# bytedance/ps-lite

Measured on AMD Instinct MI355X. Metric: push+pull GB/s per worker + p50 round-trip µs, 1 MB & 64 MB, at 1/2/4/8 GPUs, higher is better.
Workload: dtype fp32; 1 GPU; model=dense push+pull (ps-lite test_benchmark PUSH_PULL), global_batch=128, seq_len=67108864, parallelism=byteps-joint x1 (worker+server per GPU), mode=dense, msg_bytes=67108864, batch_keys=False, overlap=True, op=assign

## Files before the change

### csrc/kernels.h

```cpp
#pragma once

#include <cstddef>
#include <cstdint>

#include <hip/hip_runtime.h>

#include "coalesce_admit.h"

namespace xps {
namespace kern {

void DenseAssign(void* dst, const void* src, size_t nbytes, hipStream_t s, int grid_cap = 0);
void DenseAssign2(void* dst0, void* dst1, const void* src, size_t nbytes, hipStream_t s,
                  int grid_cap = 0);
inline bool Disjoint3(const void* a, const void* b, const void* c, size_t len) {
  auto apart = [len](const void* x, const void* y) {
    uintptr_t p = reinterpret_cast<uintptr_t>(x), q = reinterpret_cast<uintptr_t>(y);
    return p + len <= q || q + len <= p;
  };
  return apart(a, b) && apart(a, c) && apart(b, c);
}
void DenseSumF32(float* dst, const float* src, size_t n, hipStream_t s, int grid_cap = 0);
void DenseSumBf16(uint16_t* dst, const uint16_t* src, size_t n, hipStream_t s, int grid_cap = 0);
void BatchedSumBf16(const struct CopyDesc* descs_host, int n, hipStream_t s, int tile_cap = 0);
void SparseGatherF32(const float* table, const uint64_t* rows_dev, size_t nrows, size_t row_len,
                     float* out, hipStream_t s, int key_shift = 0, uint64_t row_base = 0,
                     uint64_t table_rows = ~0ull, int grid_cap = 0);
void SparseScatterAddF32(float* table, const uint64_t* rows_dev, size_t nrows, size_t row_len,
                         const float* src, bool atomic, hipStream_t s, int key_shift = 0,
                         uint64_t row_base = 0, uint64_t table_rows = ~0ull, int grid_cap = 0);
void SparseScatterAssignF32(float* table, const uint64_t* rows_dev, size_t nrows, size_t row_len,
                            const float* src, hipStream_t s, int key_shift = 0,
                            uint64_t row_base = 0, uint64_t table_rows = ~0ull,
                            int grid_cap = 0);

static const int kMaxBatch = 64;
struct CopyDesc {
  void* dst;
  const void* src;
  size_t nbytes;
};
void BatchedAssign(const CopyDesc* descs_host, int n, hipStream_t s, int tile_cap = 0);
void BatchedSumF32(const CopyDesc* descs_host, int n, hipStream_t s, int tile_cap = 0);

static_assert(kMaxBatch2 == kMaxBatch, "Seg2 batches use the batched kernels' segment limit");
void BatchedAssign2(const Seg2* segs_host, int n, hipStream_t s, int tile_cap = 0);

}
}
```

### csrc/kernels.hip

```cpp
#include <hip/hip_runtime.h>

#include <algorithm>
#include <cstdlib>

#include "kernels.h"
#include "tile_runs.h"

namespace xps {
namespace kern {

namespace {

constexpr int kBlock = 256;

inline int GridFor(size_t work_items, int cap = 8192) {
  size_t g = (work_items + kBlock - 1) / kBlock;
  if (g > static_cast<size_t>(cap)) g = cap;
  if (g == 0) g = 1;
  return static_cast<int>(g);
}

inline int CapGrid(int grid, int cap) { return cap > 0 && grid > cap ? cap : grid; }

__global__ void assign_kernel(uint4* __restrict__ dst, const uint4* __restrict__ src, size_t n4) {
  size_t i = blockIdx.x * static_cast<size_t>(blockDim.x) + threadIdx.x;
  size_t stride = static_cast<size_t>(gridDim.x) * blockDim.x;
  for (; i < n4; i += stride) dst[i] = src[i];
}

__global__ void assign_tail_kernel(char* __restrict__ dst, const char* __restrict__ src,
                                   size_t begin, size_t end) {
  size_t i = begin + blockIdx.x * static_cast<size_t>(blockDim.x) + threadIdx.x;
  size_t stride = static_cast<size_t>(gridDim.x) * blockDim.x;
  for (; i < end; i += stride) dst[i] = src[i];
}

__global__ void assign2_kernel(uint4* __restrict__ dst0, uint4* __restrict__ dst1,
                               const uint4* __restrict__ src, size_t n4, size_t tail_begin,
                               size_t nbytes) {
  size_t tid = blockIdx.x * static_cast<size_t>(blockDim.x) + threadIdx.x;
  size_t stride = static_cast<size_t>(gridDim.x) * blockDim.x;
  for (size_t i = tid; i < n4; i += stride) {
    uint4 v = src[i];
    dst0[i] = v;
    dst1[i] = v;
  }
  char* b0 = reinterpret_cast<char*>(dst0);
  char* b1 = reinterpret_cast<char*>(dst1);
  const char* bs = reinterpret_cast<const char*>(src);
  for (size_t i = tail_begin + tid; i < nbytes; i += stride) {
    char c = bs[i];
    b0[i] = c;
    b1[i] = c;
  }
}

__global__ void sum_kernel_f32(float4* __restrict__ dst, const float4* __restrict__ src,
                               size_t n4) {
  size_t i = blockIdx.x * static_cast<size_t>(blockDim.x) + threadIdx.x;
  size_t stride = static_cast<size_t>(gridDim.x) * blockDim.x;
  for (; i < n4; i += stride) {
    float4 d = dst[i];
    float4 s = src[i];
    d.x += s.x;
    d.y += s.y;
    d.z += s.z;
    d.w += s.w;
    dst[i] = d;
  }
}

__global__ void sum_tail_f32(float* __restrict__ dst, const float* __restrict__ src, size_t begin,
                             size_t end) {
  size_t i = begin + blockIdx.x * static_cast<size_t>(blockDim.x) + threadIdx.x;
  size_t stride = static_cast<size_t>(gridDim.x) * blockDim.x;
  for (; i < end; i += stride) dst[i] += src[i];
}

__device__ inline float bf16_to_f32(uint16_t h) {
  union {
    uint32_t u;
    float f;
  } c;
  c.u = static_cast<uint32_t>(h) << 16;
  return c.f;
}

// ... 58 lines not shown
                                     const float4* __restrict__ src, int shift, uint64_t base,
                                     uint64_t tab_rows) {
  size_t total = nrows * row_len4;
  size_t i = blockIdx.x * static_cast<size_t>(blockDim.x) + threadIdx.x;
  size_t stride = static_cast<size_t>(gridDim.x) * blockDim.x;
  for (; i < total; i += stride) {
    size_t r = i / row_len4;
    size_t c = i - r * row_len4;
    uint64_t row = (rows[r] >> shift) - base;
    if (row >= tab_rows) continue;
    float4* dst = table + row * row_len4 + c;
    float4 d = *dst;
    float4 v = src[i];
    d.x += v.x;
    d.y += v.y;
    d.z += v.z;
    d.w += v.w;
    *dst = d;
  }
}

__global__ void gather_rows_scalar_f32(const float* __restrict__ table,
                                       const uint64_t* __restrict__ rows, size_t nrows,
                                       size_t row_len, float* __restrict__ out, int shift,
                                       uint64_t base, uint64_t tab_rows) {
  for (size_t r = blockIdx.x; r < nrows; r += gridDim.x) {
    uint64_t row = (rows[r] >> shift) - base;
    const float* src = table + row * row_len;
    float* dst = out + r * row_len;
    for (size_t c = threadIdx.x; c < row_len; c += blockDim.x) {
      dst[c] = row < tab_rows ? src[c] : 0.f;
    }
  }
}

__global__ void scatter_assign_rows_f32(float4* __restrict__ table,
                                        const uint64_t* __restrict__ rows, size_t nrows,
                                        size_t row_len4, const float4* __restrict__ src,
                                        int shift, uint64_t base, uint64_t tab_rows) {
  size_t total = nrows * row_len4;
  size_t i = blockIdx.x * static_cast<size_t>(blockDim.x) + threadIdx.x;
  size_t stride = static_cast<size_t>(gridDim.x) * blockDim.x;
  for (; i < total; i += stride) {
    size_t r = i / row_len4;
    size_t c = i - r * row_len4;
    uint64_t row = (rows[r] >> shift) - base;
    if (row < tab_rows) table[row * row_len4 + c] = src[i];
  }
}

__global__ void scatter_assign_rows_scalar_f32(float* __restrict__ table,
                                               const uint64_t* __restrict__ rows, size_t nrows,
                                               size_t row_len, const float* __restrict__ src,
                                               int shift, uint64_t base, uint64_t tab_rows) {
  for (size_t r = blockIdx.x; r < nrows; r += gridDim.x) {
    uint64_t row = (rows[r] >> shift) - base;
    if (row >= tab_rows) continue;
    float* dst = table + row * row_len;
    const float* s = src + r * row_len;
    for (size_t c = threadIdx.x; c < row_len; c += blockDim.x) dst[c] = s[c];
  }
}

__global__ void scatter_add_rows_atomic_f32(float* __restrict__ table,
                                            const uint64_t* __restrict__ rows, size_t nrows,
                                            size_t row_len, const float* __restrict__ src,
                                            int shift, uint64_t base, uint64_t tab_rows) {
  for (size_t r = blockIdx.x; r < nrows; r += gridDim.x) {
    uint64_t row = (rows[r] >> shift) - base;
    if (row >= tab_rows) continue;
    float* dst = table + row * row_len;
    const float* s = src + r * row_len;
    for (size_t c = threadIdx.x; c < row_len; c += blockDim.x) {
      atomicAdd(&dst[c], s[c]);
    }
  }
}

struct DescArray {
  CopyDesc d[kMaxBatch];
  int n;
};

struct BalancedDescArray {
  CopyDesc d[kMaxBatch];
  unsigned long long prefix[kMaxBatch + 1];
  int n;
};

template <int kOp>
__global__ void batched_balanced_kernel(BalancedDescArray da, size_t chunks_per_block) {
  size_t total = da.prefix[da.n];
  size_t tile_begin = blockIdx.x * chunks_per_block;
  size_t tile_end = tile_begin + chunks_per_block;
  if (tile_end > total) tile_end = total;
  if (tile_begin >= total) return;
  int seg = 0;
  {
    int lo = 0, hi = da.n - 1;
    while (lo < hi) {
      int mid = (lo + hi + 1) >> 1;
      if (da.prefix[mid] <= tile_begin) {
        lo = mid;
      } else {
        hi = mid - 1;
      }
    }
    seg = lo;
  }
  for (size_t g = tile_begin + threadIdx.x; g < tile_end; g += blockDim.x) {
    while (g >= da.prefix[seg + 1]) ++seg;
    size_t local = g - da.prefix[seg];
    if (kOp == 1) {
      float4* dst = reinterpret_cast<float4*>(da.d[seg].dst) + local;
      const float4* src = reinterpret_cast<const float4*>(da.d[seg].src) + local;
      float4 a = *dst;
      float4 b = *src;
      a.x += b.x;
      a.y += b.y;
      a.z += b.z;
      a.w += b.w;
      *dst = a;
    } else if (kOp == 2) {
      uint4* dst = reinterpret_cast<uint4*>(da.d[seg].dst) + local;
      const uint4* src = reinterpret_cast<const uint4*>(da.d[seg].src) + local;
      uint4 a = *dst;
      uint4 b = *src;
      a.x = bf16x2_sum(a.x, b.x);
      a.y = bf16x2_sum(a.y, b.y);
      a.z = bf16x2_sum(a.z, b.z);
      a.w = bf16x2_sum(a.w, b.w);
      *dst = a;
    } else {
      reinterpret_cast<uint4*>(da.d[seg].dst)[local] =
          reinterpret_cast<const uint4*>(da.d[seg].src)[local];
    }
  }
}

struct Seg2Array {
  Seg2 d[kMaxBatch];
  unsigned long long prefix[kMaxBatch + 1];
  int n;
};

constexpr size_t kTileChunks2 = 512;

__global__ void __launch_bounds__(kBlock)
    batched_assign2_kernel(Seg2Array da, size_t chunks_per_block) {
  TileRunIter it = TileRunsBegin(da.prefix, da.n, chunks_per_block, blockIdx.x);
  TileRun run;
  while (TileRunsNext(da.prefix, &it, &run)) {
    uint4* __restrict__ d0 = static_cast<uint4*>(da.d[run.seg].dst0);
    uint4* __restrict__ d1 = static_cast<uint4*>(da.d[run.seg].dst1);
    const uint4* __restrict__ sp = static_cast<const uint4*>(da.d[run.seg].src);
    for (size_t i = run.lo + threadIdx.x; i < run.hi; i += kBlock) {
      uint4 v = sp[i];
      d0[i] = v;
      d1[i] = v;
    }
  }
}

__global__ void batched_assign_kernel(DescArray da) {
  for (int seg = 0; seg < da.n; ++seg) {
    uint4* dst = reinterpret_cast<uint4*>(da.d[seg].dst);
    const uint4* src = reinterpret_cast<const uint4*>(da.d[seg].src);
    size_t n4 = da.d[seg].nbytes / 16;
    size_t i = blockIdx.x * static_cast<size_t>(blockDim.x) + threadIdx.x;
    size_t stride = static_cast<size_t>(gridDim.x) * blockDim.x;
    for (; i < n4; i += stride) dst[i] = src[i];
  }
}

__global__ void batched_sum_kernel_bf16(DescArray da) {
  for (int seg = 0; seg < da.n; ++seg) {
    uint4* dst = reinterpret_cast<uint4*>(da.d[seg].dst);
    const uint4* src = reinterpret_cast<const uint4*>(da.d[seg].src);
    size_t n8 = da.d[seg].nbytes / 16;
    size_t i = blockIdx.x * static_cast<size_t>(blockDim.x) + threadIdx.x;
    size_t stride = static_cast<size_t>(gridDim.x) * blockDim.x;
    for (; i < n8; i += stride) {
      uint4 d = dst[i];
      uint4 s = src[i];
      d.x = bf16x2_sum(d.x, s.x);
      d.y = bf16x2_sum(d.y, s.y);
      d.z = bf16x2_sum(d.z, s.z);
      d.w = bf16x2_sum(d.w, s.w);
      dst[i] = d;
    }
  }
}

__global__ void batched_sum_kernel_f32(DescArray da) {
  for (int seg = 0; seg < da.n; ++seg) {
    float4* dst = reinterpret_cast<float4*>(da.d[seg].dst);
    const float4* src = reinterpret_cast<const float4*>(da.d[seg].src);
    size_t n4 = da.d[seg].nbytes / 16;
    size_t i = blockIdx.x * static_cast<size_t>(blockDim.x) + threadIdx.x;
    size_t stride = static_cast<size_t>(gridDim.x) * blockDim.x;
    for (; i < n4; i += stride) {
      float4 d = dst[i];
      float4 v = src[i];
      d.x += v.x;
      d.y += v.y;
      d.z += v.z;
      d.w += v.w;
      dst[i] = d;
    }
  }
}

}

namespace {

bool BalancedBatchEnabled() {
  static const bool on = [] {
    const char* v = getenv("XPS_BALANCED_BATCH");
    return !v || atoi(v) != 0;
  }();
  return on;
}

template <int kOp>
void LaunchBalanced(const CopyDesc* descs_host, int n, hipStream_t s, int tile_cap) {
  size_t max_blocks = tile_cap > 0 ? std::min(tile_cap, 8192) : 8192;
  for (int off = 0; off < n; off += kMaxBatch) {
    BalancedDescArray da{};
    da.n = std::min(n - off, kMaxBatch);
    unsigned long long acc = 0;
    for (int i = 0; i < da.n; ++i) {
      da.d[i] = descs_host[off + i];
      da.prefix[i] = acc;
      acc += da.d[i].nbytes / 16;
    }
    da.prefix[da.n] = acc;
    if (acc == 0) continue;
    size_t cpb = (acc + max_blocks - 1) / max_blocks;
    cpb = ((cpb + kBlock - 1) / kBlock) * kBlock;
    int grid = static_cast<int>((acc + cpb - 1) / cpb);
    hipLaunchKernelGGL((batched_balanced_kernel<kOp>), dim3(grid), dim3(kBlock), 0, s, da,
                       cpb);
  }
}

template <typename Kernel>
void LaunchLegacy(Kernel kernel, const CopyDesc* descs_host, int n, hipStream_t s,
                  int tile_cap) {
  size_t total = 0;
  for (int i = 0; i < n; ++i) total += descs_host[i].nbytes;
  if (total < 16) return;
  int grid = CapGrid(GridFor(total / 16), tile_cap);
  DescArray da{};
  for (int off = 0; off < n; off += kMaxBatch) {
    da.n = std::min(n - off, kMaxBatch);
    for (int i = 0; i < da.n; ++i) da.d[i] = descs_host[off + i];
    hipLaunchKernelGGL(kernel, dim3(grid), dim3(kBlock), 0, s, da);
  }
}

inline bool Aligned16(const void* a, const void* b) {
  return ((reinterpret_cast<uintptr_t>(a) | reinterpret_cast<uintptr_t>(b)) & 15u) == 0;
}

}

void BatchedAssign(const CopyDesc* descs_host, int n, hipStream_t s, int tile_cap) {
  if (BalancedBatchEnabled()) {
    LaunchBalanced<0>(descs_host, n, s, tile_cap);
    return;
  }
  LaunchLegacy(batched_assign_kernel, descs_host, n, s, tile_cap);
}

void BatchedAssign2(const Seg2* segs_host, int n, hipStream_t s, int tile_cap) {
  int max_blocks = tile_cap > 0 ? std::min(tile_cap, 8192) : 8192;
  int off = 0;
  while (off < n) {
    Seg2Array da{};
    unsigned long long acc = 0;
    while (off < n && da.n < kMaxBatch) {
      const Seg2& sg = segs_host[off++];
      if (sg.nbytes < 16) continue;
      da.d[da.n] = sg;
      da.prefix[da.n] = acc;
      acc += sg.nbytes / 16;
      ++da.n;
    }
    da.prefix[da.n] = acc;
    if (acc == 0) continue;
    size_t cpb = (acc + max_blocks - 1) / max_blocks;
    cpb = ((cpb + kBlock - 1) / kBlock) * kBlock;
    if (tile_cap <= 0 && cpb > kTileChunks2) cpb = kTileChunks2;
    int grid = static_cast<int>((acc + cpb - 1) / cpb);
    hipLaunchKernelGGL(batched_assign2_kernel, dim3(grid), dim3(kBlock), 0, s, da, cpb);
  }
}

void BatchedSumF32(const CopyDesc* descs_host, int n, hipStream_t s, int tile_cap) {
  if (BalancedBatchEnabled()) {
    LaunchBalanced<1>(descs_host, n, s, tile_cap);
    return;
  }
  LaunchLegacy(batched_sum_kernel_f32, descs_host, n, s, tile_cap);
}

void DenseAssign(void* dst, const void* src, size_t nbytes, hipStream_t s, int grid_cap) {
  if (!Aligned16(dst, src)) {
    if (nbytes == 0) return;
    hipLaunchKernelGGL(assign_tail_kernel, dim3(CapGrid(GridFor(nbytes), grid_cap)),
                       dim3(kBlock), 0, s, static_cast<char*>(dst),
                       static_cast<const char*>(src), size_t{0}, nbytes);
    return;
  }
  size_t n4 = nbytes / 16;
  if (n4) {
    hipLaunchKernelGGL(assign_kernel, dim3(CapGrid(GridFor(n4), grid_cap)), dim3(kBlock), 0, s,
                       static_cast<uint4*>(dst), static_cast<const uint4*>(src), n4);
  }
  if (nbytes % 16) {
    hipLaunchKernelGGL(assign_tail_kernel, dim3(1), dim3(kBlock), 0, s, static_cast<char*>(dst),
                       static_cast<const char*>(src), n4 * 16, nbytes);
  }
}

void DenseAssign2(void* dst0, void* dst1, const void* src, size_t nbytes, hipStream_t s,
                  int grid_cap) {
  if (nbytes == 0) return;
  bool aligned = ((reinterpret_cast<uintptr_t>(dst0) | reinterpret_cast<uintptr_t>(dst1) |
                   reinterpret_cast<uintptr_t>(src)) & 15u) == 0;
  size_t n4 = aligned ? nbytes / 16 : 0;
  int grid = GridFor(n4 ? n4 : nbytes);
  if (grid_cap > 0 && grid > grid_cap) grid = grid_cap;
  hipLaunchKernelGGL(assign2_kernel, dim3(grid), dim3(kBlock), 0, s, static_cast<uint4*>(dst0),
                     static_cast<uint4*>(dst1), static_cast<const uint4*>(src), n4, n4 * 16,
                     nbytes);
}

void DenseSumF32(float* dst, const float* src, size_t n, hipStream_t s, int grid_cap) {
  if (!Aligned16(dst, src)) {
    if (n == 0) return;
    hipLaunchKernelGGL(sum_tail_f32, dim3(CapGrid(GridFor(n), grid_cap)), dim3(kBlock), 0, s, dst,
                       src, size_t{0}, n);
    return;
  }
  size_t n4 = n / 4;
  if (n4) {
    hipLaunchKernelGGL(sum_kernel_f32, dim3(CapGrid(GridFor(n4), grid_cap)), dim3(kBlock), 0, s,
// ... 84 lines not shown
```

### csrc/pybind.cc

```cpp
#include <pybind11/functional.h>
#include <pybind11/numpy.h>
#include <pybind11/pybind11.h>
#include <pybind11/stl.h>

#include <atomic>
#include <thread>

#include "gpu_plane.h"
#include "hip_pool.h"
#include "hip_util.h"
#include "host_pool.h"
#include "kernels.h"
#include "kv_app.h"
#include "kv_utils.h"
#include "ps.h"
#include "server_handlers.h"
#include "shm_ring.h"
#include "simple_app.h"
#include "tile_runs.h"
#include "van.h"
#include "wire.h"

namespace py = pybind11;
using namespace xps;

namespace {

struct PoolBuffer {
  SArray<char> arr;
  uintptr_t ptr() const { return reinterpret_cast<uintptr_t>(arr.data()); }
  size_t nbytes() const { return arr.size(); }
  int device() const { return arr.device(); }
  void copy_from(py::array src) {
    py::buffer_info info = src.request();
    size_t n = static_cast<size_t>(info.size) * info.itemsize;
    XPS_CHECK_LE(n, arr.size());
    if (arr.on_device()) {
      gpu::CopyHostToDevice(arr.data(), info.ptr, n, arr.device());
    } else {
      memcpy(arr.data(), info.ptr, n);
    }
  }
  py::array_t<float> to_numpy_f32() const {
    size_t n = arr.size() / sizeof(float);
    py::array_t<float> out(n);
    if (arr.on_device()) {
      gpu::CopyDeviceToHost(out.mutable_data(), arr.data(), n * sizeof(float));
    } else {
      memcpy(out.mutable_data(), arr.data(), n * sizeof(float));
    }
    return out;
  }
};

class PyKVWorker {
 public:
  PyKVWorker(int app_id, int customer_id, int instance_idx)
      : w_(app_id, customer_id, instance_idx) {}

  int Push(py::array_t<uint64_t> keys, py::array_t<float> vals, py::array_t<int> lens) {
    SArray<Key> k;
    k.CopyFrom(keys.data(), keys.size());
    SArray<float> v;
    v.CopyFrom(vals.data(), vals.size());
    SArray<int> l;
    if (lens.size()) l.CopyFrom(lens.data(), lens.size());
    py::gil_scoped_release rel;
    return w_.ZPush(k, v, l);
  }

  py::array_t<float> PullBlocking(py::array_t<uint64_t> keys) {
    std::vector<Key> k(keys.data(), keys.data() + keys.size());
    std::vector<float> vals;
    std::vector<int> lens;
    {
      py::gil_scoped_release rel;
      int ts = w_.Pull(k, &vals, &lens);
      w_.Wait(ts);
    }
    py::array_t<float> out(vals.size());
    std::copy(vals.begin(), vals.end(), out.mutable_data());
    return out;
  }

  int ZPushPtr(py::array_t<uint64_t> keys, uintptr_t vals_ptr, size_t vals_bytes, int device,
               py::array_t<int> lens, int cmd, uintptr_t keys_dev_ptr) {
    SArray<Key> k;
    k.CopyFrom(keys.data(), keys.size());
    SArray<float> v(reinterpret_cast<float*>(vals_ptr), vals_bytes / sizeof(float), device);
    SArray<int> l;
    if (lens.size()) l.CopyFrom(lens.data(), lens.size());
    SArray<Key> kd;
    if (keys_dev_ptr) {
      kd = SArray<Key>(reinterpret_cast<Key*>(keys_dev_ptr), keys.size(), device);
    }
    py::gil_scoped_release rel;
    return w_.ZPush(k, v, l, cmd, nullptr, kd);
  }

  int ZPushPullPtr(py::array_t<uint64_t> keys, uintptr_t vals_ptr, uintptr_t out_ptr,
                   size_t vals_bytes, int device, py::array_t<int> lens, int cmd,
// ... 364 lines not shown
  m.def("kernel_on_stream", [](uintptr_t stream, uintptr_t dst, uintptr_t src, size_t n) {
    py::gil_scoped_release rel;
    kern::DenseSumF32(reinterpret_cast<float*>(dst), reinterpret_cast<float*>(src), n,
                      reinterpret_cast<hipStream_t>(stream));
    hipEvent_t ev;
    XPS_CHECK(hipEventCreateWithFlags(&ev, hipEventDisableTiming) == hipSuccess);
    XPS_CHECK(hipEventRecord(ev, reinterpret_cast<hipStream_t>(stream)) == hipSuccess);
    while (hipEventQuery(ev) != hipSuccess) {}
    (void)hipEventDestroy(ev);
  });
  m.def("ipc_open", [](py::bytes handle) {
    std::string h = handle;
    py::gil_scoped_release rel;
    hipIpcMemHandle_t hh;
    memcpy(&hh, h.data(), sizeof(hh));
    void* ptr = nullptr;
    hipError_t e = hipIpcOpenMemHandle(&ptr, hh, hipIpcMemLazyEnablePeerAccess);
    XPS_CHECK(e == hipSuccess) << "hipIpcOpenMemHandle: " << hipGetErrorString(e);
    return reinterpret_cast<uintptr_t>(ptr);
  });
  m.def("pool_in_use", []() { return HbmPool::Get()->bytes_in_use(); });
  m.def("pool_contains", [](uintptr_t p) {
    uint64_t off = 0;
    return HbmPool::Get()->OffsetOf(reinterpret_cast<const void*>(p), &off);
  });
  py::class_<PoolBuffer>(m, "PoolBuffer")
      .def_property_readonly("ptr", &PoolBuffer::ptr)
      .def_property_readonly("nbytes", &PoolBuffer::nbytes)
      .def_property_readonly("device", &PoolBuffer::device)
      .def("copy_from", &PoolBuffer::copy_from)
      .def("to_numpy_f32", &PoolBuffer::to_numpy_f32);
  m.def("pool_alloc", [](size_t nbytes) {
    PoolBuffer b;
    b.arr = HbmPool::Get()->AllocArray(nbytes);
    return b;
  });
  m.def("host_alloc", [](size_t nbytes) {
    PoolBuffer b;
    b.arr = HostShmPool::Get()->AllocArray(nbytes);
    return b;
  });

  py::class_<PyKVWorker>(m, "KVWorker")
      .def(py::init<int, int, int>(), py::arg("app_id") = 0, py::arg("customer_id") = 0,
           py::arg("instance_idx") = 0)
      .def("push", &PyKVWorker::Push, py::arg("keys"), py::arg("vals"),
           py::arg("lens") = py::array_t<int>())
      .def("pull", &PyKVWorker::PullBlocking, py::arg("keys"))
      .def("zpush_ptr", &PyKVWorker::ZPushPtr, py::arg("keys"), py::arg("vals_ptr"),
           py::arg("vals_bytes"), py::arg("device"), py::arg("lens") = py::array_t<int>(),
           py::arg("cmd") = 0, py::arg("keys_dev_ptr") = 0)
      .def("zpushpull_ptr", &PyKVWorker::ZPushPullPtr, py::arg("keys"), py::arg("vals_ptr"),
           py::arg("out_ptr"), py::arg("nbytes"), py::arg("device") = -1,
           py::arg("lens") = py::array_t<int>(), py::arg("cmd") = 0,
           py::arg("keys_dev_ptr") = 0)
      .def("zpull_ptr", &PyKVWorker::ZPullPtr, py::arg("keys"), py::arg("vals_ptr"),
           py::arg("vals_bytes"), py::arg("device"), py::arg("lens") = py::array_t<int>(),
           py::arg("cmd") = 0, py::arg("keys_dev_ptr") = 0)
      .def("wait", &PyKVWorker::Wait)
      .def("round", &PyKVWorker::Round, py::arg("keys"), py::arg("ptrs"), py::arg("nbytes"),
           py::arg("device"), py::arg("cmd") = 0, py::arg("pull") = false)
      .def("round_mixed", &PyKVWorker::RoundMixed, py::arg("keys"), py::arg("push_ptrs"),
           py::arg("pull_ptrs"), py::arg("sizes"), py::arg("device"), py::arg("cmd") = 0,
           py::arg("overlap") = true);

  py::class_<PyKVServer>(m, "KVServer")
      .def(py::init<int, int>(), py::arg("app_id") = 0, py::arg("instance_idx") = 0)
      .def("set_default_handle", &PyKVServer::SetDefaultHandle)
      .def("set_reduce_handle", &PyKVServer::SetReduceHandle, py::arg("num_workers"))
      .def("set_gpu_dense_handle", &PyKVServer::SetGpuDenseHandle, py::arg("mode") = "assign",
           py::arg("dtype") = "f32")
      .def("set_gpu_sparse_handle", &PyKVServer::SetGpuSparseHandle, py::arg("rows"),
           py::arg("row_len"), py::arg("accumulate") = true, py::arg("key_shift") = 0)
      .def("register_entry", &PyKVServer::RegisterEntry, py::arg("key"), py::arg("ptr"),
           py::arg("nbytes"), py::arg("device") = 0)
      .def("sparse_table_ptr", &PyKVServer::SparseTablePtr)
      .def("save_checkpoint", &PyKVServer::SaveCheckpoint)
      .def("load_checkpoint", &PyKVServer::LoadCheckpoint)
      .def("set_python_handle", &PyKVServer::SetPythonHandle);

  m.def("zero_copy_recv_count", []() { return g_zero_copy_recv.load(); });
  m.def("fused_assign_count", []() { return g_fused_assign.load(); });
  m.def("fused_assign_launches", []() { return g_fused_launches.load(); });
  m.def("coalesce_admit",
        [](const std::vector<std::tuple<uintptr_t, uintptr_t, uintptr_t, size_t>>& open,
           const std::tuple<uintptr_t, uintptr_t, uintptr_t, size_t>& seg) {
          auto conv = [](const std::tuple<uintptr_t, uintptr_t, uintptr_t, size_t>& t) {
            return kern::Seg2{reinterpret_cast<void*>(std::get<0>(t)),
                              reinterpret_cast<void*>(std::get<1>(t)),
                              reinterpret_cast<const void*>(std::get<2>(t)), std::get<3>(t)};
          };
          std::vector<kern::Seg2> segs;
          for (auto& t : open) segs.push_back(conv(t));
          switch (kern::CoalesceAdmit(segs.data(), static_cast<int>(segs.size()), conv(seg))) {
            case kern::Admit::kAdmit: return "admit";
            case kern::Admit::kFlushFirst: return "flush";
            default: return "reject";
          }
        },
        py::arg("open"), py::arg("seg"));
  m.def("tile_runs",
        [](const std::vector<unsigned long long>& chunk_counts,
           unsigned long long chunks_per_block, unsigned long long block_index) {
          if (chunks_per_block == 0) throw std::invalid_argument("tile_runs: empty tile");
          std::vector<unsigned long long> prefix(chunk_counts.size() + 1, 0);
          for (size_t i = 0; i < chunk_counts.size(); ++i) {
            if (chunk_counts[i] == 0) throw std::invalid_argument("tile_runs: empty segment");
            prefix[i + 1] = prefix[i] + chunk_counts[i];
          }
          int n = static_cast<int>(chunk_counts.size());
          std::vector<std::tuple<int, unsigned long long, unsigned long long>> out;
          kern::TileRunIter it = kern::TileRunsBegin(prefix.data(), n, chunks_per_block,
                                                     block_index);
          kern::TileRun run;
          while (kern::TileRunsNext(prefix.data(), &it, &run)) {
            out.emplace_back(run.seg, run.lo, run.hi);
          }
          return out;
        },
        py::arg("chunk_counts"), py::arg("chunks_per_block"), py::arg("block_index"));

  m.def("plane_peer_bytes", [](const std::string& role, int idx) {
    py::dict out;
    auto* po = GetPO(role, idx);
    auto* plane = po->van() ? dynamic_cast<GpuPlane*>(po->van()->plane()) : nullptr;
    if (plane) {
      for (auto& t : plane->PeerBytes()) {
        out[py::int_(std::get<0>(t))] = py::make_tuple(std::get<1>(t), std::get<2>(t));
      }
    }
    return out;
  }, py::arg("role") = "worker", py::arg("idx") = 0);

  m.def("_order_nodes", [](std::vector<std::tuple<std::string, std::string, int>> in) {
    std::vector<Node> nodes;
    for (auto& t : in) {
      Node n;
      n.role = std::get<0>(t) == "worker" ? Node::WORKER : Node::SERVER;
      n.hostname = std::get<1>(t);
      n.port = std::get<2>(t);
      nodes.push_back(n);
    }
    auto less = NodeRankOrder(nodes);
    std::sort(nodes.begin(), nodes.end(), less);
    std::vector<std::tuple<std::string, std::string, int>> out;
    for (auto& n : nodes) {
      out.emplace_back(n.role == Node::WORKER ? "worker" : "server", n.hostname, n.port);
    }
    return out;
  });

  m.def("_host_pool_init_for_test", [](uint64_t uid, size_t bytes) {
    HostShmPool::Get()->Init(uid, bytes);
  });
  m.def("_gc_stale_shm", []() { HostShmPool::GcStaleSegments(); });

  m.def("_ring_stress", [](int producers, int per, int payload) {
    ShmRing ring;
    XPS_CHECK(ring.Create(0xabcdef12345ull + getpid()));
    std::atomic<long> received{0}, sum{0}, pushed{0};
    std::atomic<bool> done{false};
    std::thread consumer([&]() {
      std::vector<char> buf(ShmRing::MaxPayload());
      while (true) {
        uint32_t n = ring.Pop(buf.data());
        if (n == 0) {
// ... 301 lines not shown
```

### csrc/server_handlers.cc

```cpp
#include "server_handlers.h"

#include "gpu_plane.h"
#include "hip_pool.h"
#include "kernels.h"

namespace xps {

#define XPS_HIP_CHECK(cmd)                                                            \
  do {                                                                                \
    hipError_t e_ = (cmd);                                                            \
    XPS_CHECK(e_ == hipSuccess) << "HIP error: " << hipGetErrorString(e_) << " in " #cmd; \
  } while (0)

static GpuPlane* ThePlane(Postoffice* po) {
  return dynamic_cast<GpuPlane*>(po->van() ? po->van()->plane() : nullptr);
}

static hipStream_t PeerStream(Postoffice* po, int sender, hipStream_t* fallback) {
  auto* plane = ThePlane(po);
  if (plane) return plane->StreamForPeer(sender);
  if (!*fallback) {
    XPS_HIP_CHECK(hipStreamCreateWithFlags(fallback, hipStreamNonBlocking));
  }
  return *fallback;
// ... 126 lines not shown
  }
  if (e->buf.size() != len) return false;
  const char* src = reinterpret_cast<const char*>(kvs.vals.data());
  if (!kern::Disjoint3(e->buf.data(), dst, src, len)) return false;
  bool chain = NeedChain(req.sender);
  bool coalesced = !chain && !e->last_ev &&
                   plane->CoalesceAppend(req.sender, kern::Seg2{e->buf.data(), dst, src, len});
  if (!coalesced) {
    hipStream_t stream = Stream(req.sender);
    OrderAfter(e, stream);
    kern::DenseAssign2(e->buf.data(), dst, src, len, stream);
    g_fused_launches.fetch_add(1, std::memory_order_relaxed);
    if (chain) e->last_ev = MakeEventRef(po_, stream);
  }
  g_fused_assign.fetch_add(1, std::memory_order_relaxed);
  g_zero_copy_recv.fetch_add(1, std::memory_order_relaxed);
  KVMeta r = req;
  r.option |= kOptInPlace;
  r.option &= ~(kOptPullLane | kOptEntryPush);
  r.val_len = static_cast<int64_t>(len);
  uint64_t eoff = 0;
  if (HbmPool::Get()->OffsetOf(e->buf.data(), &eoff)) {
    r.entry_addr = eoff;
    r.option |= kOptEntryAddr;
  }
  server->Response(r);
  if (coalesced) plane->CoalesceEnd(req.sender);
  return true;
}

GpuDenseHandler::Group* GpuDenseHandler::GroupFor(const SArray<Key>& keys) {
  uint64_t h = 1469598103934665603ull;
  const unsigned char* p = reinterpret_cast<const unsigned char*>(keys.data());
  for (size_t i = 0; i < keys.nbytes(); ++i) {
    h ^= p[i];
    h *= 1099511628211ull;
  }
  Group* g;
  {
    std::lock_guard<std::mutex> lk(mu_);
    g = &groups_[h];
  }
  if (g->keys.empty()) {
    g->keys.assign(keys.begin(), keys.end());
    g->ents.reserve(keys.size());
    std::lock_guard<std::mutex> lk(mu_);
    for (Key k : g->keys) g->ents.push_back(&store_[k]);
  } else {
    XPS_CHECK(g->keys.size() == keys.size() &&
              std::equal(g->keys.begin(), g->keys.end(), keys.begin()))
        << "reduce mode needs a consistent key->message grouping across workers "
           "(key-set hash collision or inconsistent bucketing)";
  }
  return g;
}

void GpuDenseHandler::HandleReducePush(const KVMeta& req, const KVPairs<float>& kvs,
                                       KVServer<float>* server) {
  XPS_STAGE(reduce_push);
  size_t n = kvs.keys.size();
  Group* g = GroupFor(kvs.keys);
  if (g->pushes >= num_workers_) {
    g->waiting_pushes.emplace_back(req, kvs);
    return;
  }
  XPS_CHECK(kvs.vals.on_device()) << "reduce mode needs device vals (pool buffers)";
  if (g->lens.size() != n) {
    g->lens.resize(n);
    for (size_t i = 0; i < n; ++i) {
      g->lens[i] = kvs.lens.empty() ? kvs.vals.nbytes() / n
                                    : static_cast<size_t>(kvs.lens[i]) * sizeof(float);
    }
  }
  hipStream_t stream = Stream(req.sender);
  XPS_HIP_CHECK(hipSetDevice(HbmPool::Get()->device()));
  if (g->last_ev) XPS_HIP_CHECK(hipStreamWaitEvent(stream, g->last_ev.get(), 0));
  bool first = g->pushes == 0;
  if (first) {
    for (auto& ev : g->pull_guard) {
      XPS_HIP_CHECK(hipStreamWaitEvent(stream, ev.get(), 0));
    }
    g->pull_guard.clear();
  }
  std::vector<kern::CopyDesc> descs;
  descs.reserve(n);
  size_t off = 0;
  bool aligned = true;
  for (size_t i = 0; i < n; ++i) {
    size_t len = g->lens[i];
    Entry* e = g->ents[i];
    if (e->buf.size() < len) e->buf = HbmPool::Get()->AllocArray(len);
    descs.push_back({e->buf.data(), reinterpret_cast<const char*>(kvs.vals.data()) + off, len});
    aligned = aligned && (len % 16 == 0);
    off += len;
  }
  if (aligned) {
    if (first) {
      kern::BatchedAssign(descs.data(), static_cast<int>(n), stream);
    } else {
      BatchedSum(descs.data(), static_cast<int>(n), stream);
    }
  } else {
    for (auto& d : descs) {
      if (first) {
        kern::DenseAssign(d.dst, d.src, d.nbytes, stream);
      } else {
        SumKernel(d.dst, d.src, d.nbytes, stream);
      }
    }
  }
  g->pushes++;
  EventRef ev = MakeEventRef(po_, stream);
  g->round_events.push_back(ev);
  g->last_ev = ev;
  server->Response(req);
  if (g->pushes >= num_workers_) {
    std::vector<KVMeta> waiting;
    waiting.swap(g->waiting_pulls);
    for (auto& w : waiting) RespondPull(w, g, server);
  }
}

void GpuDenseHandler::HandlePush(const KVMeta& req, const KVPairs<float>& kvs,
                                 KVServer<float>* server, bool respond) {
  XPS_STAGE(dense_push);
  size_t n = kvs.keys.size();
  XPS_CHECK_GT(n, 0u);
  if (mode_ == DenseMode::kReduce) {
    HandleReducePush(req, kvs, server);
    return;
  }
  if (req.option & kOptInPlace) {
    if (respond) server->Response(req);
    return;
  }
  hipStream_t stream = Stream(req.sender);
  XPS_HIP_CHECK(hipSetDevice(HbmPool::Get()->device()));
  bool chain = NeedChain(req.sender);
  bool sum_all = mode_ == DenseMode::kAssign ? req.cmd == kCmdSum : req.cmd != kCmdAssign;
  if (kvs.vals.on_device() && n > 1) {
    std::vector<kern::CopyDesc> descs;
    std::vector<Entry*> ents;
    descs.reserve(n);
    ents.reserve(n);
    size_t boff = 0;
    bool aligned = true;
    for (size_t i = 0; i < n; ++i) {
      size_t len = kvs.lens.empty() ? kvs.vals.nbytes() / n
                                    : static_cast<size_t>(kvs.lens[i]) * sizeof(float);
      Entry* e;
      {
        std::lock_guard<std::mutex> lk(mu_);
        e = &store_[kvs.keys[i]];
        if (e->buf.size() < len) {
          e->buf = HbmPool::Get()->AllocArray(len);
          XPS_HIP_CHECK(hipMemset(e->buf.data(), 0, len));
        }
      }
      ents.push_back(e);
      descs.push_back({e->buf.data(),
                       reinterpret_cast<const char*>(kvs.vals.data()) + boff, len});
      aligned = aligned && (len % 16 == 0) && (boff % 16 == 0);
      boff += len;
    }
    if (aligned) {
      for (Entry* e : ents) OrderAfter(e, stream);
      if (sum_all) {
        BatchedSum(descs.data(), static_cast<int>(n), stream);
      } else {
        kern::BatchedAssign(descs.data(), static_cast<int>(n), stream);
      }
      if (chain) {
        EventRef ev = MakeEventRef(po_, stream);
        for (Entry* e : ents) e->last_ev = ev;
      }
      auto* plane0 = po_->van() ? po_->van()->plane() : nullptr;
      if (!plane0) XPS_HIP_CHECK(hipStreamSynchronize(stream));
      if (respond) server->Response(req);
      return;
    }
  }
  size_t off = 0;
  bool synced = false;
  Entry* last_e = nullptr;
  for (size_t i = 0; i < n; ++i) {
    size_t len = kvs.lens.empty() ? kvs.vals.nbytes() / n
                                  : static_cast<size_t>(kvs.lens[i]) * sizeof(float);
    Entry* e;
    {
      std::lock_guard<std::mutex> lk(mu_);
      e = &store_[kvs.keys[i]];
      if (e->buf.size() < len) {
        if (!e->buf.empty()) e->retired.push_back(e->buf);
        e->buf = HbmPool::Get()->AllocArray(len);
        XPS_HIP_CHECK(hipMemset(e->buf.data(), 0, len));
      }
    }
    last_e = e;
    bool sum = sum_all;
    const char* src = reinterpret_cast<const char*>(kvs.vals.data()) + off;
    if (kvs.vals.on_device()) {
      OrderAfter(e, stream);
      {
        XPS_STAGE(push_kernel_launch);
        if (sum) {
          SumKernel(e->buf.data(), src, len, stream);
        } else {
          kern::DenseAssign(e->buf.data(), src, len, stream);
        }
      }
      if (chain) {
        XPS_STAGE(push_chain_event);
        e->last_ev = MakeEventRef(po_, stream);
      }
    } else {
      if (chain && e->last_ev) {
        XPS_HIP_CHECK(hipEventSynchronize(e->last_ev.get()));
        e->last_ev.reset();
      }
      if (sum) {
        SArray<char> scratch = HbmPool::Get()->AllocArray(len);
        XPS_HIP_CHECK(hipMemcpy(scratch.data(), src, len, hipMemcpyHostToDevice));
        SumKernel(e->buf.data(), scratch.data(), len, stream);
        XPS_HIP_CHECK(hipStreamSynchronize(stream));
        synced = true;
      } else {
        XPS_HIP_CHECK(hipMemcpy(e->buf.data(), src, len, hipMemcpyHostToDevice));
      }
    }
    off += len;
  }
  auto* plane = po_->van() ? po_->van()->plane() : nullptr;
  if (!plane && !synced) XPS_HIP_CHECK(hipStreamSynchronize(stream));
  if (!respond) return;
  if (mode_ == DenseMode::kAssign && n == 1 && last_e && plane) {
    uint64_t eoff = 0;
    if (HbmPool::Get()->OffsetOf(last_e->buf.data(), &eoff)) {
      KVMeta r = req;
      r.addr = eoff;
      r.val_len = static_cast<int64_t>(last_e->buf.size());
      r.option |= kOptEntryAddr;
      server->Response(r);
      return;
    }
  }
  server->Response(req);
}

void GpuDenseHandler::RespondPull(const KVMeta& req, Group* g, KVServer<float>* server) {
  XPS_STAGE(reduce_respond_pull);
  hipStream_t stream = PullStream(req.sender);
  for (auto& ev : g->round_events) {
    XPS_HIP_CHECK(hipStreamWaitEvent(stream, ev.get(), 0));
  }
  size_t n = g->keys.size();
  size_t total = 0;
  for (size_t len : g->lens) total += len;
  SArray<Key> keys(g->keys);
  SArray<int> lens(n);
  for (size_t i = 0; i < n; ++i) lens[i] = static_cast<int>(g->lens[i] / sizeof(float));
  bool responded = false;
  if (req.option & kOptPullAddr) {
    if (auto* plane = ThePlane(po_)) {
      std::vector<kern::CopyDesc> descs;
      descs.reserve(n);
      uint64_t off = 0;
      bool ok = true;
      for (size_t i = 0; i < n && ok; ++i) {
        size_t len = g->lens[i];
        char* dst = plane->PeerDst(req.sender, req.addr + off, len);
        ok = dst != nullptr && len % 16 == 0;
        if (ok) {
          descs.push_back({dst, g->ents[i]->buf.data(), len});
          off += len;
        }
      }
      if (ok) {
        kern::BatchedAssign(descs.data(), static_cast<int>(n), stream);
        KVMeta r2 = req;
        r2.option |= kOptInPlace | kOptPullLane;
        r2.val_len = static_cast<int64_t>(total);
        KVPairs<float> res2;
        res2.keys = keys;
        res2.lens = lens;
        server->Response(r2, res2);
        responded = true;
      }
    }
  }
  if (!responded) {
    KVPairs<float> res;
    res.keys = keys;
    res.lens = lens;
    if (n == 1) {
      res.vals = SArray<float>::View(g->ents[0]->buf);
    } else {
      SArray<char> tmp = HbmPool::Get()->AllocArray(total);
      std::vector<kern::CopyDesc> descs;
      descs.reserve(n);
      size_t off = 0;
      bool aligned = true;
      for (size_t i = 0; i < n; ++i) {
        descs.push_back({tmp.data() + off, g->ents[i]->buf.data(), g->lens[i]});
        aligned = aligned && (g->lens[i] % 16 == 0) && (off % 16 == 0);
        off += g->lens[i];
      }
      if (aligned) {
        kern::BatchedAssign(descs.data(), static_cast<int>(n), stream);
      } else {
        for (auto& d : descs) kern::DenseAssign(d.dst, d.src, d.nbytes, stream);
      }
      res.vals = SArray<float>::View(tmp);
    }
    if (!(req.option & kOptPullAddr)) XPS_HIP_CHECK(hipStreamSynchronize(stream));
    KVMeta r = req;
    r.option |= kOptPullLane;
    server->Response(r, res);
  }
  EventRef pe = MakeEventRef(po_, stream);
  g->pull_guard.push_back(pe);
  g->last_ev = pe;
  g->pulled_senders.insert(req.sender);
  g->pulls++;
  if (g->pulls >= num_workers_) {
    g->pushes = 0;
    g->pulls = 0;
    g->pulled_senders.clear();
    g->round_events.clear();
    std::vector<std::pair<KVMeta, KVPairs<float>>> dpush;
    dpush.swap(g->waiting_pushes);
    for (auto& d : dpush) HandleReducePush(d.first, d.second, server);
    std::vector<KVMeta> dpull;
    dpull.swap(g->waiting_next_pulls);
    for (auto& d : dpull) {
      if (g->pushes >= num_workers_) {
        RespondPull(d, g, server);
      } else {
        g->waiting_pulls.push_back(d);
      }
    }
  }
}

void GpuDenseHandler::HandlePull(const KVMeta& req, const KVPairs<float>& kvs,
                                 KVServer<float>* server) {
  XPS_STAGE(dense_pull);
  size_t n = kvs.keys.size();
  XPS_CHECK_GT(n, 0u);
  XPS_HIP_CHECK(hipSetDevice(HbmPool::Get()->device()));
  if (mode_ == DenseMode::kReduce) {
    Group* g = GroupFor(kvs.keys);
    if (g->pulled_senders.count(req.sender)) {
      g->waiting_next_pulls.push_back(req);
      return;
    }
    if (g->pushes < num_workers_) {
      g->waiting_pulls.push_back(req);
      return;
    }
    RespondPull(req, g, server);
    return;
  }
  hipStream_t stream = PullStream(req.sender);
  bool chain = NeedChain(req.sender);
  if (n > 1 && (req.option & kOptPullAddr)) {
    if (auto* plane = ThePlane(po_)) {
      std::vector<kern::CopyDesc> descs;
      std::vector<Entry*> ents;
      SArray<int> lens2(n);
      uint64_t off = 0;
      bool ok = true;
      {
        std::lock_guard<std::mutex> lk(mu_);
        for (size_t i = 0; i < n && ok; ++i) {
          auto it = store_.find(kvs.keys[i]);
          XPS_CHECK(it != store_.end()) << "pull of unknown key " << kvs.keys[i];
          size_t len = it->second.buf.size();
          char* dst = plane->PeerDst(req.sender, req.addr + off, len);
          ok = dst != nullptr && len % 16 == 0 && off % 16 == 0;
          if (ok) {
            ents.push_back(&it->second);
            descs.push_back({dst, it->second.buf.data(), len});
// ... 251 lines not shown
```

### csrc/server_handlers.h

```cpp
#pragma once

#include <hip/hip_runtime.h>

#include <memory>
#include <set>
#include <type_traits>
#include <unordered_map>

#include "kernels.h"
#include "kv_app.h"

namespace xps {

using EventRef = std::shared_ptr<std::remove_pointer<hipEvent_t>::type>;

enum class DenseMode {
  kAssign,
  kSum,
  kReduce,
};

enum class DenseDtype { kF32, kBf16 };

class GpuDenseHandler {
 public:
  GpuDenseHandler(Postoffice* po, DenseMode mode, DenseDtype dtype = DenseDtype::kF32);
  ~GpuDenseHandler();
  void operator()(const KVMeta& req, const KVPairs<float>& kvs, KVServer<float>* server);

  void Save(const std::string& path);
  void Load(const std::string& path);

  void RegisterEntry(Key key, void* ptr, size_t nbytes, int device);

 private:
  struct Entry {
    SArray<char> buf;
    EventRef last_ev;
    std::vector<SArray<char>> retired;
  };

  struct Group {
    std::vector<Key> keys;
    std::vector<Entry*> ents;
    std::vector<size_t> lens;
    int pushes = 0;
    int pulls = 0;
    std::vector<KVMeta> waiting_pulls;
    std::vector<std::pair<KVMeta, KVPairs<float>>> waiting_pushes;
    std::vector<KVMeta> waiting_next_pulls;
    std::set<int> pulled_senders;
    std::vector<EventRef> round_events;
    std::vector<EventRef> pull_guard;
    EventRef last_ev;
  };

  void HandlePush(const KVMeta& req, const KVPairs<float>& kvs, KVServer<float>* server,
                  bool respond = true);
  bool TryFusedAssign(const KVMeta& req, const KVPairs<float>& kvs, KVServer<float>* server);
  void HandleReducePush(const KVMeta& req, const KVPairs<float>& kvs, KVServer<float>* server);
  void HandlePull(const KVMeta& req, const KVPairs<float>& kvs, KVServer<float>* server);
  void RespondPull(const KVMeta& req, Group* g, KVServer<float>* server);
  Group* GroupFor(const SArray<Key>& keys);
  hipStream_t Stream(int sender);
  hipStream_t PullStream(int sender);
  bool NeedChain(int sender);
  void OrderAfter(Entry* e, hipStream_t s);

  void SumKernel(void* dst, const void* src, size_t nbytes, hipStream_t s);
  void BatchedSum(const kern::CopyDesc* descs, int n, hipStream_t s);

  Postoffice* po_;
  DenseMode mode_;
  DenseDtype dtype_;
  int num_workers_ = 1;
  bool chain_ = false;
  std::mutex mu_;
  std::unordered_map<Key, Entry> store_;
  std::unordered_map<uint64_t, Group> groups_;
  hipStream_t fallback_stream_ = nullptr;
};

class GpuSparseHandler {
 public:
  GpuSparseHandler(Postoffice* po, size_t rows, size_t row_len, bool accumulate,
                   int key_shift = 0);
  void operator()(const KVMeta& req, const KVPairs<float>& kvs, KVServer<float>* server);
  uintptr_t table_ptr() const { return reinterpret_cast<uintptr_t>(table_.data()); }
  void Save(const std::string& path);
  void Load(const std::string& path);

 private:
  hipStream_t Stream(int sender);
  const uint64_t* DeviceKeys(const SArray<Key>& keys, int sender, hipStream_t s);

  Postoffice* po_;
  size_t rows_;
  size_t row_len_;
  bool accumulate_;
  bool atomic_ = false;
  int key_shift_ = 0;
  uint64_t row_base_ = 0;
  SArray<char> table_;
  std::mutex mu_;
  std::unordered_map<int, SArray<char>> key_scratch_;
  hipStream_t fallback_stream_ = nullptr;
};

}
```

### csrc/tile_runs.h

```cpp
#pragma once

#include <cstddef>
#include <cstdint>

#if defined(__HIPCC__)
#define XPS_HOST_DEVICE __host__ __device__
#else
#define XPS_HOST_DEVICE
#endif

namespace xps {
namespace kern {

struct TileRun {
  int seg;
  unsigned long long lo, hi;
};

struct TileRunIter {
  int seg;
  unsigned long long pos, end;
};

XPS_HOST_DEVICE inline TileRunIter TileRunsRange(const unsigned long long* prefix, int n,
                                                 unsigned long long begin,
                                                 unsigned long long end) {
  TileRunIter it;
  unsigned long long total = prefix[n];
  it.end = end < total ? end : total;
  it.pos = begin;
  it.seg = 0;
  if (it.pos >= it.end) {
    it.pos = it.end;
    return it;
  }
  int lo = 0, hi = n - 1;
  while (lo < hi) {
    int mid = (lo + hi + 1) >> 1;
    if (prefix[mid] <= begin) {
      lo = mid;
    } else {
      hi = mid - 1;
    }
  }
  it.seg = lo;
  return it;
}

XPS_HOST_DEVICE inline TileRunIter TileRunsBegin(const unsigned long long* prefix, int n,
                                                 unsigned long long chunks_per_block,
                                                 unsigned long long block_index) {
  unsigned long long begin = block_index * chunks_per_block;
  return TileRunsRange(prefix, n, begin, begin + chunks_per_block);
}

XPS_HOST_DEVICE inline bool TileRunsNext(const unsigned long long* prefix, TileRunIter* it,
                                         TileRun* run) {
  if (it->pos >= it->end) return false;
  unsigned long long seg_lo = prefix[it->seg], seg_hi = prefix[it->seg + 1];
  unsigned long long stop = seg_hi < it->end ? seg_hi : it->end;
  run->seg = it->seg;
  run->lo = it->pos - seg_lo;
  run->hi = stop - seg_lo;
  it->pos = stop;
  ++it->seg;
  return true;
}

}
}
```

Baseline: 3922 GB/s.

## Widen balanced batch kernel to 192 segments and cache per-group pull metadata

```diff
diff --git a/csrc/batch_split.h b/csrc/batch_split.h
--- /dev/null
+++ b/csrc/batch_split.h
@@ -0,0 +1,33 @@
+#pragma once
+
+#include <cstddef>
+#include <cstdint>
+
+namespace xps {
+namespace kern {
+
+struct BatchSpan {
+  int begin, end;
+  int nseg;
+  unsigned long long chunks;
+};
+
+template <typename ChunkAt>
+inline BatchSpan NextBatch(ChunkAt chunk_at, int n, int begin, int max_segs,
+                           unsigned long long max_chunks) {
+  BatchSpan b{begin, begin, 0, 0};
+  while (b.end < n) {
+    unsigned long long c = chunk_at(b.end);
+    if (c != 0) {
+      if (b.nseg >= max_segs) break;
+      if (b.nseg > 0 && (c > max_chunks || b.chunks > max_chunks - c)) break;
+      b.chunks += c;
+      ++b.nseg;
+    }
+    ++b.end;
+  }
+  return b;
+}
+
+}
+}
diff --git a/csrc/kernels.h b/csrc/kernels.h
--- a/csrc/kernels.h
+++ b/csrc/kernels.h
@@ -40,8 +40,11 @@
   const void* src;
   size_t nbytes;
 };
+static const int kMaxBatchWide = 192;
 void BatchedAssign(const CopyDesc* descs_host, int n, hipStream_t s, int tile_cap = 0);
 void BatchedSumF32(const CopyDesc* descs_host, int n, hipStream_t s, int tile_cap = 0);
+uint64_t BatchedLaunches();
+int BalancedMaxSegs();
 
 static_assert(kMaxBatch2 == kMaxBatch, "Seg2 batches use the batched kernels' segment limit");
 void BatchedAssign2(const Seg2* segs_host, int n, hipStream_t s, int tile_cap = 0);
diff --git a/csrc/kernels.hip b/csrc/kernels.hip
--- a/csrc/kernels.hip
+++ b/csrc/kernels.hip
@@ -1,8 +1,11 @@
 #include <hip/hip_runtime.h>
 
 #include <algorithm>
+#include <atomic>
+#include <cstdio>
 #include <cstdlib>
 
+#include "batch_split.h"
 #include "kernels.h"
 #include "tile_runs.h"
 
@@ -227,58 +230,54 @@
   int n;
 };
 
-struct BalancedDescArray {
-  CopyDesc d[kMaxBatch];
-  unsigned long long prefix[kMaxBatch + 1];
+struct WideSeg {
+  void* dst;
+  const void* src;
+};
+struct WideDescArray {
+  WideSeg d[kMaxBatchWide];
+  uint32_t prefix[kMaxBatchWide + 1];
   int n;
 };
+static_assert(sizeof(WideDescArray) + sizeof(size_t) <= 4096,
+              "WideDescArray and chunks_per_block must fit the kernel-argument limit");
+
+constexpr size_t kTileChunksWide = 512;
 
 template <int kOp>
-__global__ void batched_balanced_kernel(BalancedDescArray da, size_t chunks_per_block) {
-  size_t total = da.prefix[da.n];
-  size_t tile_begin = blockIdx.x * chunks_per_block;
-  size_t tile_end = tile_begin + chunks_per_block;
-  if (tile_end > total) tile_end = total;
-  if (tile_begin >= total) return;
-  int seg = 0;
-  {
-    int lo = 0, hi = da.n - 1;
-    while (lo < hi) {
-      int mid = (lo + hi + 1) >> 1;
-      if (da.prefix[mid] <= tile_begin) {
-        lo = mid;
-      } else {
-        hi = mid - 1;
+__global__ void __launch_bounds__(kBlock)
+    batched_balanced_kernel(WideDescArray da, size_t chunks_per_block) {
+  TileRunIter it = TileRunsBegin(da.prefix, da.n, chunks_per_block, blockIdx.x);
+  TileRun run;
+  while (TileRunsNext(da.prefix, &it, &run)) {
+    if (kOp == 1) {
+      float4* __restrict__ dst = static_cast<float4*>(da.d[run.seg].dst);
+      const float4* __restrict__ src = static_cast<const float4*>(da.d[run.seg].src);
+      for (size_t i = run.lo + threadIdx.x; i < run.hi; i += kBlock) {
+        float4 a = dst[i];
+        float4 b = src[i];
+        a.x += b.x;
+        a.y += b.y;
+        a.z += b.z;
+        a.w += b.w;
+        dst[i] = a;
       }
-    }
-    seg = lo;
-  }
-  for (size_t g = tile_begin + threadIdx.x; g < tile_end; g += blockDim.x) {
-    while (g >= da.prefix[seg + 1]) ++seg;
-    size_t local = g - da.prefix[seg];
-    if (kOp == 1) {
-      float4* dst = reinterpret_cast<float4*>(da.d[seg].dst) + local;
-      const float4* src = reinterpret_cast<const float4*>(da.d[seg].src) + local;
-      float4 a = *dst;
-      float4 b = *src;
-      a.x += b.x;
-      a.y += b.y;
-      a.z += b.z;
-      a.w += b.w;
-      *dst = a;
     } else if (kOp == 2) {
-      uint4* dst = reinterpret_cast<uint4*>(da.d[seg].dst) + local;
-      const uint4* src = reinterpret_cast<const uint4*>(da.d[seg].src) + local;
-      uint4 a = *dst;
-      uint4 b = *src;
-      a.x = bf16x2_sum(a.x, b.x);
-      a.y = bf16x2_sum(a.y, b.y);
-      a.z = bf16x2_sum(a.z, b.z);
-      a.w = bf16x2_sum(a.w, b.w);
-      *dst = a;
+      uint4* __restrict__ dst = static_cast<uint4*>(da.d[run.seg].dst);
+      const uint4* __restrict__ src = static_cast<const uint4*>(da.d[run.seg].src);
+      for (size_t i = run.lo + threadIdx.x; i < run.hi; i += kBlock) {
+        uint4 a = dst[i];
+        uint4 b = src[i];
+        a.x = bf16x2_sum(a.x, b.x);
+        a.y = bf16x2_sum(a.y, b.y);
+        a.z = bf16x2_sum(a.z, b.z);
+        a.w = bf16x2_sum(a.w, b.w);
+        dst[i] = a;
+      }
     } else {
-      reinterpret_cast<uint4*>(da.d[seg].dst)[local] =
-          reinterpret_cast<const uint4*>(da.d[seg].src)[local];
+      uint4* __restrict__ dst = static_cast<uint4*>(da.d[run.seg].dst);
+      const uint4* __restrict__ src = static_cast<const uint4*>(da.d[run.seg].src);
+      for (size_t i = run.lo + threadIdx.x; i < run.hi; i += kBlock) dst[i] = src[i];
     }
   }
 }
@@ -368,25 +367,48 @@
   return on;
 }
 
+bool WideBatchEnabled() {
+  static const bool on = [] {
+    const char* v = getenv("XPS_WIDE_BATCH");
+    return !v || atoi(v) != 0;
+  }();
+  return on;
+}
+
+std::atomic<uint64_t> g_batched_launches{0};
+
 template <int kOp>
 void LaunchBalanced(const CopyDesc* descs_host, int n, hipStream_t s, int tile_cap) {
   size_t max_blocks = tile_cap > 0 ? std::min(tile_cap, 8192) : 8192;
-  for (int off = 0; off < n; off += kMaxBatch) {
-    BalancedDescArray da{};
-    da.n = std::min(n - off, kMaxBatch);
-    unsigned long long acc = 0;
-    for (int i = 0; i < da.n; ++i) {
-      da.d[i] = descs_host[off + i];
-      da.prefix[i] = acc;
-      acc += da.d[i].nbytes / 16;
+  auto chunk_at = [descs_host](int i) -> unsigned long long { return descs_host[i].nbytes / 16; };
+  int max_segs = BalancedMaxSegs();
+  for (int off = 0; off < n;) {
+    BatchSpan span = NextBatch(chunk_at, n, off, max_segs, UINT32_MAX);
+    off = span.end;
+    if (span.nseg == 0) continue;
+    if (span.chunks > UINT32_MAX) {
+      fprintf(stderr, "xps: batched segment of %llu chunks exceeds the 32-bit chunk prefix\n",
+              span.chunks);
+      abort();
+    }
+    WideDescArray da{};
+    uint32_t acc = 0;
+    for (int i = span.begin; i < span.end; ++i) {
+      size_t chunks = descs_host[i].nbytes / 16;
+      if (chunks == 0) continue;
+      da.d[da.n] = WideSeg{descs_host[i].dst, descs_host[i].src};
+      da.prefix[da.n] = acc;
+      acc += static_cast<uint32_t>(chunks);
+      ++da.n;
     }
     da.prefix[da.n] = acc;
-    if (acc == 0) continue;
     size_t cpb = (acc + max_blocks - 1) / max_blocks;
     cpb = ((cpb + kBlock - 1) / kBlock) * kBlock;
+    if (tile_cap <= 0 && cpb > kTileChunksWide) cpb = kTileChunksWide;
     int grid = static_cast<int>((acc + cpb - 1) / cpb);
     hipLaunchKernelGGL((batched_balanced_kernel<kOp>), dim3(grid), dim3(kBlock), 0, s, da,
                        cpb);
+    g_batched_launches.fetch_add(1, std::memory_order_relaxed);
   }
 }
 
@@ -402,6 +424,7 @@
     da.n = std::min(n - off, kMaxBatch);
     for (int i = 0; i < da.n; ++i) da.d[i] = descs_host[off + i];
     hipLaunchKernelGGL(kernel, dim3(grid), dim3(kBlock), 0, s, da);
+    g_batched_launches.fetch_add(1, std::memory_order_relaxed);
   }
 }
 
@@ -410,6 +433,10 @@
 }
 
 }
+
+uint64_t BatchedLaunches() { return g_batched_launches.load(std::memory_order_relaxed); }
+
+int BalancedMaxSegs() { return WideBatchEnabled() ? kMaxBatchWide : kMaxBatch; }
 
 void BatchedAssign(const CopyDesc* descs_host, int n, hipStream_t s, int tile_cap) {
   if (BalancedBatchEnabled()) {
diff --git a/csrc/pybind.cc b/csrc/pybind.cc
--- a/csrc/pybind.cc
+++ b/csrc/pybind.cc
@@ -17,6 +17,7 @@
 #include "server_handlers.h"
 #include "shm_ring.h"
 #include "simple_app.h"
+#include "batch_split.h"
 #include "tile_runs.h"
 #include "van.h"
 #include "wire.h"
@@ -547,6 +548,25 @@
   m.def("zero_copy_recv_count", []() { return g_zero_copy_recv.load(); });
   m.def("fused_assign_count", []() { return g_fused_assign.load(); });
   m.def("fused_assign_launches", []() { return g_fused_launches.load(); });
+  m.def("batched_launches", []() { return kern::BatchedLaunches(); });
+  m.attr("kMaxBatch") = kern::kMaxBatch;
+  m.attr("kMaxBatchWide") = kern::kMaxBatchWide;
+  m.def("batch_split",
+        [](const std::vector<unsigned long long>& chunk_counts, int max_segs,
+           unsigned long long max_chunks) {
+          if (max_segs < 1) throw std::invalid_argument("batch_split: max_segs < 1");
+          int n = static_cast<int>(chunk_counts.size());
+          auto chunk_at = [&chunk_counts](int i) { return chunk_counts[i]; };
+          std::vector<std::tuple<int, int, int, unsigned long long>> out;
+          for (int off = 0; off < n;) {
+            kern::BatchSpan b = kern::NextBatch(chunk_at, n, off, max_segs, max_chunks);
+            off = b.end;
+            if (b.nseg) out.emplace_back(b.begin, b.end, b.nseg, b.chunks);
+          }
+          return out;
+        },
+        py::arg("chunk_counts"), py::arg("max_segs") = kern::kMaxBatchWide,
+        py::arg("max_chunks") = 0xFFFFFFFFull);
   m.def("coalesce_admit",
         [](const std::vector<std::tuple<uintptr_t, uintptr_t, uintptr_t, size_t>>& open,
            const std::tuple<uintptr_t, uintptr_t, uintptr_t, size_t>& seg) {
diff --git a/csrc/server_handlers.cc b/csrc/server_handlers.cc
--- a/csrc/server_handlers.cc
+++ b/csrc/server_handlers.cc
@@ -232,15 +232,16 @@
     }
     g->pull_guard.clear();
   }
-  std::vector<kern::CopyDesc> descs;
-  descs.reserve(n);
+  std::vector<kern::CopyDesc>& descs = g->descs;
+  descs.clear();
   size_t off = 0;
   bool aligned = true;
+  const char* vals = reinterpret_cast<const char*>(kvs.vals.data());
   for (size_t i = 0; i < n; ++i) {
     size_t len = g->lens[i];
     Entry* e = g->ents[i];
     if (e->buf.size() < len) e->buf = HbmPool::Get()->AllocArray(len);
-    descs.push_back({e->buf.data(), reinterpret_cast<const char*>(kvs.vals.data()) + off, len});
+    descs.push_back({e->buf.data(), vals + off, len});
     aligned = aligned && (len % 16 == 0);
     off += len;
   }
@@ -404,22 +405,33 @@
     XPS_HIP_CHECK(hipStreamWaitEvent(stream, ev.get(), 0));
   }
   size_t n = g->keys.size();
-  size_t total = 0;
-  for (size_t len : g->lens) total += len;
-  SArray<Key> keys(g->keys);
-  SArray<int> lens(n);
-  for (size_t i = 0; i < n; ++i) lens[i] = static_cast<int>(g->lens[i] / sizeof(float));
+  if (g->resp_keys.size() != n) {
+    g->resp_keys = SArray<Key>(g->keys);
+    SArray<int> rl(n);
+    g->total = 0;
+    g->all16 = true;
+    for (size_t i = 0; i < n; ++i) {
+      rl[i] = static_cast<int>(g->lens[i] / sizeof(float));
+      g->total += g->lens[i];
+      g->all16 = g->all16 && g->lens[i] % 16 == 0;
+    }
+    g->resp_lens = rl;
+  }
+  size_t total = g->total;
+  const SArray<Key>& keys = g->resp_keys;
+  const SArray<int>& lens = g->resp_lens;
+  std::vector<kern::CopyDesc>& descs = g->descs;
   bool responded = false;
   if (req.option & kOptPullAddr) {
     if (auto* plane = ThePlane(po_)) {
-      std::vector<kern::CopyDesc> descs;
-      descs.reserve(n);
+      descs.clear();
+      bool ok = g->all16;
+      char* base = ok ? plane->PeerDst(req.sender, req.addr, total) : nullptr;
       uint64_t off = 0;
-      bool ok = true;
       for (size_t i = 0; i < n && ok; ++i) {
         size_t len = g->lens[i];
-        char* dst = plane->PeerDst(req.sender, req.addr + off, len);
-        ok = dst != nullptr && len % 16 == 0;
+        char* dst = base ? base + off : plane->PeerDst(req.sender, req.addr + off, len);
+        ok = dst != nullptr;
         if (ok) {
           descs.push_back({dst, g->ents[i]->buf.data(), len});
           off += len;
@@ -446,8 +458,7 @@
       res.vals = SArray<float>::View(g->ents[0]->buf);
     } else {
       SArray<char> tmp = HbmPool::Get()->AllocArray(total);
-      std::vector<kern::CopyDesc> descs;
-      descs.reserve(n);
+      descs.clear();
       size_t off = 0;
       bool aligned = true;
       for (size_t i = 0; i < n; ++i) {
diff --git a/csrc/server_handlers.h b/csrc/server_handlers.h
--- a/csrc/server_handlers.h
+++ b/csrc/server_handlers.h
@@ -44,6 +44,11 @@
     std::vector<Key> keys;
     std::vector<Entry*> ents;
     std::vector<size_t> lens;
+    SArray<Key> resp_keys;
+    SArray<int> resp_lens;
+    size_t total = 0;
+    bool all16 = false;
+    std::vector<kern::CopyDesc> descs;
     int pushes = 0;
     int pulls = 0;
     std::vector<KVMeta> waiting_pulls;
diff --git a/csrc/tile_runs.h b/csrc/tile_runs.h
--- a/csrc/tile_runs.h
+++ b/csrc/tile_runs.h
@@ -22,7 +22,8 @@
   unsigned long long pos, end;
 };
 
-XPS_HOST_DEVICE inline TileRunIter TileRunsRange(const unsigned long long* prefix, int n,
+template <typename Prefix>
+XPS_HOST_DEVICE inline TileRunIter TileRunsRange(const Prefix* prefix, int n,
                                                  unsigned long long begin,
                                                  unsigned long long end) {
   TileRunIter it;
@@ -47,15 +48,16 @@
   return it;
 }
 
-XPS_HOST_DEVICE inline TileRunIter TileRunsBegin(const unsigned long long* prefix, int n,
+template <typename Prefix>
+XPS_HOST_DEVICE inline TileRunIter TileRunsBegin(const Prefix* prefix, int n,
                                                  unsigned long long chunks_per_block,
                                                  unsigned long long block_index) {
   unsigned long long begin = block_index * chunks_per_block;
   return TileRunsRange(prefix, n, begin, begin + chunks_per_block);
 }
 
-XPS_HOST_DEVICE inline bool TileRunsNext(const unsigned long long* prefix, TileRunIter* it,
-                                         TileRun* run) {
+template <typename Prefix>
+XPS_HOST_DEVICE inline bool TileRunsNext(const Prefix* prefix, TileRunIter* it, TileRun* run) {
   if (it->pos >= it->end) return false;
   unsigned long long seg_lo = prefix[it->seg], seg_hi = prefix[it->seg + 1];
   unsigned long long stop = seg_hi < it->end ? seg_hi : it->end;
```

After: 3966 GB/s, median of 5. 1.1% higher.
